# zaiisao/ConTEXTure-NeRF

Measured on AMD Instinct MI355X. Metric: UNet denoise steps/sec (CFG-batched SD2-depth UNet eval + PLMS update), higher is better.
Workload: dtype f16; 1 GPU; BASELINE configs[1]: 1 view @768^2 (latent 96^2), 50 PLMS steps (51 UNet evals), SD2-depth UNet fp16, CFG batch 2, guidance 10, random-init weights; mesh substitution napoleon.obj -> n/a for this stage (denoise loop only); latent=96, cfg_batch=2, ctx_len=77, views_per_rank=1, parallelism=view-shard x1

## Files before the change

contexture-nerf_amd/_lib.py:

```python
import ctypes as C
import os
import torch

_HERE = os.path.dirname(os.path.abspath(__file__))
LIB_PATH = os.path.join(_HERE, "libctxnerf.so")

_vp, _i32, _i64, _f32 = C.c_void_p, C.c_int32, C.c_int64, C.c_float

SIGNATURES = {
    "ctx_version": (_i32, []),
    "ctx_last_error": (C.c_char_p, []),
    "ctx_device_check": (_i32, []),
    "ctx_prepare_vertices": (_i32, [_vp, _vp, _vp, _vp, _i32, _i32, _i32, _vp, _vp, _vp, _vp, _vp]),
    "ctx_rasterize_ws_bytes": (_i64, [_i32, _i32, _i32, _i32]),
    "ctx_rasterize_fwd": (_i32, [_i32, _i32, _vp, _vp, _vp, _i32, _i32, _i32, _f32, _f32, _vp, _vp, _vp, _i64, _vp]),
    "ctx_rasterize_fused": (_i32, [_i32, _i32, _vp, _vp, _vp, _i32, _vp, _i32, _i32, _f32, _f32, _vp, _vp, _vp, _vp, _vp, _i64, _vp]),
    "ctx_normalize_depth_ws_bytes": (_i64, [_i32]),
    "ctx_normalize_depth": (_i32, [_vp, _i32, _i32, _vp, _vp, _vp, _vp]),
    "ctx_texture_mapping_fwd": (_i32, [_vp, _vp, _i32, _i32, _i32, _i32, _i32, _i32, _vp, _vp, _vp]),
    "ctx_texture_mapping_bwd": (_i32, [_vp, _vp, _i32, _i32, _i32, _i32, _vp, _vp, _vp]),
    "ctx_texmap_bwd_plan_bytes": (_i64, [_i32, _i32, _i32]),
    "ctx_texmap_bwd_plan": (_i32, [_vp, _vp, _i32, _i32, _i32, _vp, _vp]),
    "ctx_texture_mapping_bwd_binned_ws_bytes": (_i64, [_i32, _i32]),
    "ctx_texture_mapping_bwd_binned": (_i32, [_vp, _vp, _vp, _i32, _i32, _i32, _i32, _vp, _vp, _vp, _vp]),
    "ctx_texmap_plan_max_res": (_i32, []),
    "ctx_texmap_plan_stale": (_i32, [_vp, _vp]),
    "ctx_uv_scatter_fixed": (_i32, [_vp, _vp, _vp, _i32, _i32, _i32, _i32, _vp, _i32, _vp, _vp]),
    "ctx_fixed_to_float": (_i32, [_vp, _i64, _i32, _i32, _vp, _vp]),
    "ctx_uv_gather_ws_bytes": (_i64, [_i32, _i32]),
    "ctx_uv_gather_fixed": (_i32, [_vp, _vp, _vp, _vp, _vp, _vp, _vp, _i32, _i32, _i32, _i32, _i32, _i32, _i32, _vp, _vp, _i64, _vp]),
    "ctx_atlas_fill_ws_bytes": (_i64, [_i32]),
    "ctx_nearest_seed": (_i32, [_vp, _i32, _vp, _vp, _vp, _i64, _vp]),
    "ctx_atlas_fill": (_i32, [_vp, _vp, _vp, _i32, _i32, _i32, _vp, _vp, _vp, _i64, _vp]),
    "ctx_view_consistency_ws_bytes": (_i64, [_i32, _i32]),
    "ctx_view_consistency_fwd": (_i32, [_vp, _vp, _vp, _vp, _i32, _i32, _i32, _i32, _i32, _i32, _i32, _i32, _vp, _i64, _vp, _vp, _vp, _vp, _vp]),
    "ctx_view_consistency_bwd": (_i32, [_vp, _vp, _vp, _vp, _vp, _i32, _i32, _i32, _i32, _i32, _i32, _i32, _vp, _vp, _vp, _vp, _vp]),
    "ctx_texture_pack4": (_i32, [_vp, _i32, _i32, _vp, _vp]),
    "ctx_texture_mapping_packed_fwd": (_i32, [_vp, _vp, _i32, _i32, _i32, _i32, _i32, _vp, _vp, _vp]),
    "ctx_view_weights_max": (_i32, [_vp, _vp, _i32, _i32, _i32, _vp, _vp, _vp]),
    "ctx_view_weights_mask": (_i32, [_vp, _vp, _vp, _i32, _i32, _i32, _vp, _vp]),
    "ctx_face_view_map_ws_bytes": (_i64, [_i32, _i32, _i32]),
    "ctx_face_view_map": (_i32, [_vp, _i32, _i32, _i32, _vp, _vp, _vp, _vp]),
    "ctx_embed_fwd": (_i32, [_vp, _i64, _i32, _i32, _vp, _vp]),
    "ctx_uvmlp_packed_bytes": (_i64, [_i32, _i32, _i32, _i32, _i32]),
    "ctx_uvmlp_pack": (_i32, [_vp, _vp, _i32, _i32, _i32, _i32, _i32, _vp, _vp]),
    "ctx_uvmlp_fwd": (_i32, [_vp, _vp, _i64, _i32, _vp, _i32, _i32, _i32, _i32, _i32, _vp, _vp, _vp]),
    "ctx_uvmlp_saved_bytes": (_i64, [_i64, _i32, _i32, _i32]),
    "ctx_uvmlp_fwd_save": (_i32, [_vp, _vp, _i64, _i32, _vp, _i32, _i32, _i32, _i32, _i32, _i32, _vp, _vp, _vp, _vp]),
    "ctx_uvmlp_bwd_ws_bytes": (_i64, [_i64, _i32, _i32]),
    "ctx_uvmlp_bwd": (_i32, [_vp, _vp, _vp, _i64, _vp, _i32, _i32, _i32, _i32, _i32, _i32, _vp, _vp, _vp, _vp, _vp]),
    "ctx_uvmlp_fwd_emb": (_i32, [_vp, _i64, _vp, _i32, _i32, _i32, _i32, _i32, _vp, _vp, _vp]),
    "ctx_uvmlp_bwd_emb": (_i32, [_vp, _i64, _vp, _i32, _i32, _i32, _i32, _i32, _vp, _vp, _vp, _vp, _vp, _vp]),
    "ctx_texel_active_mark": (_i32, [_vp, _vp, _i32, _i32, _i32, _i32, _vp, _vp]),
    "ctx_texel_compact_ws_bytes": (_i64, [_i64]),
    "ctx_texel_compact": (_i32, [_vp, _i64, _vp, _vp, _vp, _vp]),
    "ctx_uvmlp_fwd_save_idx": (_i32, [_vp, _i64, _i32, _vp, _i32, _i32, _i32, _i32, _i32, _vp, _vp, _vp, _vp]),
    "ctx_uvmlp_bwd_idx": (_i32, [_vp, _vp, _vp, _i32, _vp, _i64, _vp, _i32, _i32, _i32, _i32, _i32, _vp, _vp, _vp, _vp, _vp]),
    "ctx_get_rays": (_i32, [_i32, _i32, _f32, _f32, _f32, _f32, _vp, _vp, _vp, _vp]),
    "ctx_raymarch_composite_fwd": (_i32, [_vp, _vp, _vp, _i64, _i32, _i32, _vp, _vp, _vp, _vp, _vp, _vp]),
    "ctx_raymarch_composite_fwd_noise": (_i32, [_vp, _vp, _vp, _vp, _i64, _i32, _i32, _vp, _vp, _vp, _vp, _vp, _vp]),
    "ctx_raymarch_composite_bwd": (_i32, [_vp, _vp, _vp, _vp, _i64, _i32, _i32, _vp, _vp, _vp, _vp, _vp, _vp, _vp]),
    "ctx_occ_mark": (_i32, [_vp, _vp, _vp, _i64, _i32, _vp, _i32, _f32, _f32, _f32, _f32, _f32, _f32, _vp, _vp]),
    "ctx_occ_points": (_i32, [_vp, _vp, _vp, _i64, _i32, _vp, _i64, _vp, _vp]),
    "ctx_occ_expand": (_i32, [_vp, _vp, _i64, _i64, _vp, _vp]),
    "ctx_occ_collect": (_i32, [_vp, _vp, _i64, _i64, _vp, _vp]),
    "ctx_occ_cell_points": (_i32, [_i32, _f32, _f32, _f32, _f32, _f32, _f32, _vp, _vp, _vp]),
    "ctx_occ_update": (_i32, [_vp, _vp, _vp, _i64, _f32, _f32, _vp]),
    "ctx_occ_voxelize": (_i32, [_vp, _vp, _i64, _i64, _i32, _f32, _f32, _f32, _f32, _f32, _f32, _vp, _vp]),
    "ctx_occ_dilate": (_i32, [_vp, _i32, _i32, _vp, _vp, _vp]),
    "ctx_occ_ray_spans": (_i32, [_vp, _vp, _i64, _f32, _f32, _vp, _i32, _f32, _f32, _f32, _f32, _f32, _f32, _f32, _f32, _f32, _f32, _f32, _f32,
                                 _vp, _vp, _vp]),
    "ctx_occ_march_count": (_i32, [_vp, _vp, _i64, _f32, _f32, _vp, _i32] + [_f32] * 13 + [_vp, _vp]),
    "ctx_occ_march_write": (_i32, [_vp, _vp, _i64, _f32, _f32, _vp, _i32] + [_f32] * 13 + [_vp, _vp, _i64, _vp, _vp, _vp, _vp, _vp]),
    "ctx_raymarch_packed_fwd": (_i32, [_vp, _vp, _vp, _vp, _vp, _vp, _i64, _i64, _i32, _vp, _vp, _vp, _vp, _vp, _vp]),
    "ctx_raymarch_packed_bwd": (_i32, [_vp, _vp, _vp, _vp, _vp, _vp, _i64, _i64, _i32, _vp, _vp, _vp, _vp, _vp, _vp, _vp]),
    "ctx_distortion_packed_fwd": (_i32, [_vp, _vp, _vp, _vp, _vp, _i64, _i64, _vp, _vp]),
    "ctx_distortion_packed_bwd": (_i32, [_vp, _vp, _vp, _vp, _vp, _i64, _i64, _vp, _vp, _vp]),
    "ctx_resample_packed": (_i32, [_vp, _vp, _vp, _vp, _vp, _vp, _i64, _i64, _i32, _vp, _vp, _i64, _vp, _vp, _vp, _vp, _vp]),
    "ctx_hashgrid_fwd": (_i32, [_vp, _i64, _vp, _i32, _i32, _i32, _vp, _vp, _vp, _vp, _vp]),
    "ctx_hashgrid_bwd_ws_bytes": (_i64, [_i32, _i32, _i32]),
    "ctx_hashgrid_bwd": (_i32, [_vp, _i64, _vp, _i32, _i32, _i32, _vp, _vp, _vp, _i32, _vp, _vp, _vp]),
    "ctx_hashgrid_bwd_pts_ws_bytes": (_i64, [_i64, _i32]),
    "ctx_hashgrid_bwd_pts": (_i32, [_vp, _i64, _vp, _vp, _i32, _i32, _i32, _vp, _vp, _vp, _vp, _vp, _vp]),
    "ctx_hashtex_fwd": (_i32, [_vp, _vp, _i64, _i32, _vp, _i32, _i32, _i32, _vp, _vp, _vp]),
    "ctx_hashtex_bwd_ws_bytes": (_i64, [_i32, _i32, _i32]),
    "ctx_hashtex_bwd": (_i32, [_vp, _vp, _i64, _i32, _vp, _i32, _i32, _i32, _vp, _i32, _vp, _vp, _vp]),
    "ctx_texture_head_fwd": (_i32, [_vp, _vp, _i64, _i64, _i32, _vp, _vp]),
    "ctx_texture_head_bwd": (_i32, [_vp, _vp, _vp, _vp, _i64, _i64, _i32, _vp, _vp]),
    "ctx_weighted_sum_packed": (_i32, [_vp, _vp, _vp, _i64, _i64, _i32, _vp, _vp]),
    "ctx_unet_create": (_vp, [_vp]),
    "ctx_unet_destroy": (None, [_vp]),
    "ctx_unet_param_count": (_i32, [_vp]),
    "ctx_unet_param_name": (C.c_char_p, [_vp, _i32]),
    "ctx_unet_param_shape": (_i32, [_vp, _i32, _vp]),
    "ctx_unet_weight_bytes": (_i64, [_vp]),
    "ctx_unet_workspace_bytes": (_i64, [_vp, _i32, _i32, _i32, _i32]),
    "ctx_unet_bind": (_i32, [_vp, _vp, _vp, _i64]),
    "ctx_unet_set_param": (_i32, [_vp, _i32, _vp, _vp]),
    "ctx_unet_forward": (_i32, [_vp, _vp, _vp, _vp, _i32, _i32, _i32, _i32, _vp, _vp]),
    "ctx_controlnet_create": (_vp, [_vp, _i32]),
    "ctx_controlnet_residual_bytes": (_i64, [_vp, _i32, _i32, _i32]),
    "ctx_controlnet_cond_cache_bytes": (_i64, [_vp, _i32, _i32, _i32]),
    "ctx_controlnet_forward": (_i32, [_vp, _vp, _vp, _vp, _vp, _vp, _i32, _i32, _i32, _i32, _i32, _vp, _vp]),
    "ctx_unet_set_residuals": (_i32, [_vp, _vp, C.c_float]),
    "ctx_unet_ref_bank_bytes": (_i64, [_vp, _i32, _i32, _i32]),
    "ctx_unet_workspace_bytes_ref": (_i64, [_vp, _i32, _i32, _i32, _i32, _i32, _i32]),
    "ctx_unet_forward_ref": (_i32, [_vp, _vp, _vp, _vp, _i32, _i32, _i32, _i32, _i32, _vp, _i32, _vp, _vp]),
    "ctx_unet_set_residual_fp32": (_i32, [_vp, _i32]),
    "ctx_unet_stats": (_i32, [_vp, _i32, _vp, _vp]),
    "ctx_unet_gn_epilogue_counts": (_i32, [_vp, _vp, _vp]),
    "ctx_unet_set_taps": (_i32, [_vp, _vp, _i64]),
    "ctx_unet_tap_count": (_i32, [_vp]),
    "ctx_unet_tap_info": (_i32, [_vp, _i32, _vp, _vp, _vp]),
    "ctx_vae_create": (_vp, [_vp]),
    "ctx_vae_destroy": (None, [_vp]),
    "ctx_vae_param_count": (_i32, [_vp]),
    "ctx_vae_param_name": (C.c_char_p, [_vp, _i32]),
    "ctx_vae_param_shape": (_i32, [_vp, _i32, _vp]),
    "ctx_vae_weight_bytes": (_i64, [_vp]),
    "ctx_vae_workspace_bytes": (_i64, [_vp, _i32, _i32, _i32]),
    "ctx_vae_bind": (_i32, [_vp, _vp, _vp, _i64]),
    "ctx_vae_set_param": (_i32, [_vp, _i32, _vp, _vp]),
    "ctx_vae_decode": (_i32, [_vp, _vp, _i32, _i32, _i32, _vp, _vp]),
    "ctx_vae_decoder_param_count": (_i32, [_vp]),
    "ctx_vae_encode_workspace_bytes": (_i64, [_vp, _i32, _i32, _i32]),
    "ctx_vae_encode": (_i32, [_vp, _vp, _i32, _i32, _i32, _vp, _vp]),
    "ctx_vae_flops": (C.c_double, [_vp]),
    "ctx_vae_encode_train_workspace_bytes": (_i64, [_vp, _i32, _i32, _i32]),
    "ctx_vae_encode_train": (_i32, [_vp, _vp, _i32, _i32, _i32, _vp, _vp]),
    "ctx_vae_encode_bwd": (_i32, [_vp, _vp, _f32, _vp, _vp]),
    "ctx_gemm_f16": (_i32, [_vp, _vp, _vp, _vp, _i32, _i32, _i32, _vp, _vp]),
    "ctx_conv3x3_f16": (_i32, [_vp, _vp, _vp, _vp, _vp, _i32, _i32, _i32, _i32, _i32, _i32, _i32, _vp, _vp]),
    "ctx_conv3x3_seg_f16": (_i32, [_vp, _vp, _vp, _vp, _vp, _vp, _i32, _i32, _i32, _i32, _i32, _vp, _vp, _i32, _i32, _vp, _vp, _i32, _i32,
                                   _vp, _i32, _vp, _vp]),
    "ctx_conv3x3_gn_f16": (_i32, [_vp, _vp, _vp, _vp, _vp, _vp, _i32, _i32, _i32, _i32, _i32, _vp, _i32, _i32, _i32, _vp, _vp, _vp, _vp]),
    "ctx_gemm_last_kernel": (None, [_vp, _vp]),
    "ctx_conv3x3_geom_f16": (_i32, [_vp, _vp, _vp, _vp, _i32, _i32, _i32, _i32, _i32, _i32, _i32, _i32, _i32, _vp, _i32, _vp, _vp]),
    "ctx_pack_conv3_dgrad_f16": (_i32, [_vp, _i32, _i32, _i32, _vp, _vp]),
    "ctx_pack_mat_dgrad_f16": (_i32, [_vp, _i32, _i32, _i32, _i32, _vp, _vp]),
    "ctx_groupnorm_bwd_ws_bytes": (_i64, [_i32, _i32]),
    "ctx_groupnorm_bwd_f16": (_i32, [_vp, _vp, _vp, _vp, _vp, _i32, _i32, _i32, _i32, _f32, _i32, _vp, _vp, _vp]),
    "ctx_softmax_rows_f16": (_i32, [_vp, _i32, _i32, _f32, _vp, _vp]),
    "ctx_softmax_bwd_rows_f16": (_i32, [_vp, _vp, _i32, _i32, _f32, _vp, _vp]),
    "ctx_quant_bwd_f16": (_i32, [_vp, _vp, _i32, _i32, _i64, _f32, _vp, _vp]),
    "ctx_conv_in_bwd_f16": (_i32, [_vp, _vp, _i32, _i32, _i32, _i32, _i32, _f32, _vp, _vp]),
    "ctx_conv_in_f16": (_i32, [_vp, _vp, _vp, _i32, _i32, _i32, _i32, _i32, _vp, _vp]),
    "ctx_conv_out_f16": (_i32, [_vp, _vp, _vp, _i32, _i32, _i32, _i32, _i32, _vp, _vp]),
    "ctx_gemv_f16": (_i32, [_vp, _vp, _vp, _i32, _i32, _i32, _i32, _i32, _vp, _vp]),
    "ctx_time_embed_f16": (_i32, [_vp, _i32, _i32, _vp, _vp]),
    "ctx_transpose_v_f16": (_i32, [_vp, _i32, _i32, _i32, _i32, _i32, _vp, _vp]),
    "ctx_concat_f16": (_i32, [_vp, _vp, _i64, _i32, _i32, _vp, _vp]),
    "ctx_concat_f32": (_i32, [_vp, _vp, _i64, _i32, _i32, _vp, _vp]),
    "ctx_f32_to_f16": (_i32, [_vp, _i64, _vp, _vp]),
    "ctx_f16_to_f32": (_i32, [_vp, _i64, _vp, _vp]),
    "ctx_conv_small_f16": (_i32, [_vp, _vp, _vp, _vp, _i32, _i32, _i32, _i32, _i32, _i32, _i32, _vp, _vp]),
    "ctx_add_scaled_f16": (_i32, [_vp, _vp, _f32, _i64, _vp]),
    "ctx_pointwise_f32": (_i32, [_vp, _vp, _vp, _i32, _i32, _i64, _i32, _vp, _vp]),
    "ctx_pack_fwd_f16": (_i32, [_vp, _i32, _i32, _i32, _vp, _vp]),
    "ctx_groupnorm_f16": (_i32, [_vp, _vp, _vp, _i32, _i32, _i32, _i32, _f32, _i32, _vp, _vp, _vp]),
    "ctx_groupnorm2_f16": (_i32, [_vp, _vp, _i32, _vp, _vp, _i32, _i32, _i32, _i32, _f32, _i32, _vp, _vp, _vp]),
    "ctx_groupnorm_apply_f16": (_i32, [_vp, _vp, _i32, _vp, _vp, _i32, _i32, _i32, _i32, _f32, _i32, _vp, _vp]),
    "ctx_groupnorm_slabs_f16": (_i32, [_vp, _i32, _vp, _vp, _vp, _i32, _vp, _vp, _i32, _i32, _i32, _i32, _f32, _i32, _vp, _vp]),
    "ctx_layernorm_f16": (_i32, [_vp, _vp, _vp, _i64, _i32, _f32, _vp, _vp]),
    "ctx_attention_ws_bytes": (_i64, [_i32, _i32, _i32]),
    "ctx_attention_f16": (_i32, [_vp, _vp, _vp, _i32, _i32, _i32, _i32, _i32, _i32, _f32, _vp, _i32, _vp, _vp]),
    "ctx_groupnorm_ws_bytes": (_i64, [_i32, _i32]),
    "ctx_geglu_f16": (_i32, [_vp, _i64, _i32, _vp, _vp]),
    "ctx_profile_begin": (_i32, []),
    "ctx_profile_end": (_i32, [_i32, _vp, _vp]),
    "ctx_bench_gemm": (C.c_float, [_vp, _vp, _vp, _vp, _i32, _i32, _i32, _vp, _i32, _i32, _i32, _i32, _i32, _i32, _vp, _i32, _i32, _vp]),
    "ctx_gemm_tune": (None, [_i32, _i32]),
    "ctx_attention_tune": (None, [_i32, _i32, _i32, _f32]),
    "ctx_probe_mfma": (_i32, [_i32, _vp, _vp, _vp, _vp]),
    "ctx_probe_stage": (C.c_float, [_i32, _i32, _i32, _i32, _i32, _vp, _vp, _vp]),
    "ctx_cfg_plms_step": (_i32, [_vp, _i64, _f32, _vp, _i32, _vp, _f32, _f32, _i32, _vp, _vp, _vp]),
}


class CtxError(RuntimeError):
    pass


_lib = None


def load():
    global _lib
    if _lib is None:
        if not os.path.exists(LIB_PATH):
            raise CtxError(f"{LIB_PATH} is missing: run `python -c 'import __graft_entry__ as g; g.build()'` "
                           "(hipcc --offload-arch=gfx950). There is no CPU fallback for this path.")
        lib = C.CDLL(LIB_PATH)
        for name, (res, args) in SIGNATURES.items():
            if not hasattr(lib, name) and os.environ.get("CTX_ALLOW_PARTIAL") == "1":
                continue
            fn = getattr(lib, name)
            fn.restype = res
            fn.argtypes = args
        _lib = lib
    return _lib


def check(rc):
    if rc != 0:
        raise CtxError(f"libctxnerf error {rc}: {load().ctx_last_error().decode()}")


def stream():
    return C.c_void_p(torch.cuda.current_stream().cuda_stream)


def ptr(t, dtype=None, name="tensor"):
    if t is None:
        return C.c_void_p(0)
    if not isinstance(t, torch.Tensor) or not t.is_cuda:
        raise CtxError(f"{name}: expected a device tensor (the HIP path has no CPU fallback), got "
                       f"{type(t).__name__} on {getattr(t, 'device', '?')}")
    if not t.is_contiguous():
        raise CtxError(f"{name}: tensor must be contiguous")
    if dtype is not None and t.dtype != dtype:
        raise CtxError(f"{name}: expected dtype {dtype}, got {t.dtype}")
    return C.c_void_p(t.data_ptr())


def f32c(t, device=None):
    t = t.to(dtype=torch.float32)
    if device is not None:
        t = t.to(device)
    return t.contiguous()
```

contexture-nerf_amd/csrc/attention.hip:

```cpp
#include "gemm_common.h"
#include <math.h>

#define AT_KB 64
#define AT_KROW 72
#define AT_VROW 68


struct AttnArgs {
    const f16 *Q, *K, *V;
    f16 *O;
    int Sq, Skv, heads;
    int q_stride, kv_stride, o_stride;
    float scale_log2e;
    float lazy;
};



typedef short at_s16x4 __attribute__((__vector_size__(4 * sizeof(short))));
__device__ __forceinline__ f16x4 at_tr16(const f16 *p)
{
    at_s16x4 v = __builtin_amdgcn_ds_read_tr16_b64_v4i16((__attribute__((address_space(3))) at_s16x4 *)p);
    return __builtin_bit_cast(f16x4, v);
}
struct AtNoIssue { __device__ __forceinline__ void operator()(int) const {} };
template <bool MASK, int NISSUE = 0, class Issue = AtNoIssue>
__device__ __forceinline__ void attn_tile(const f16 *__restrict__ Ks, const f16 *__restrict__ Vs, int k0, int Skv, int r, int h,
                                          int swz, int vlane, int vfq, float c, const f16x8 (&qf)[4], f32x16 (&o)[2], f32x16 &ls,
                                          float &m_run, float lazy, Issue iss = Issue())
{
    f32x16 s[2];
#pragma unroll
    for (int kb = 0; kb < 2; ++kb) {
#pragma unroll
        for (int q = 0; q < 16; ++q) s[kb][q] = 0.f;
        const f16 *kr = Ks + (kb * 32 + r) * 64;
#pragma unroll
        for (int ks = 0; ks < 4; ++ks) {
            f16x8 kf = *(const f16x8 *)(kr + ((2 * ks + h) ^ swz) * 8);
            s[kb] = __builtin_amdgcn_mfma_f32_32x32x16_f16(kf, qf[ks], s[kb], 0, 0, 0);
            if (kb * 4 + ks < NISSUE) iss(kb * 4 + ks);
        }
    }
    if (MASK) {
#pragma unroll
        for (int kb = 0; kb < 2; ++kb)
#pragma unroll
            for (int q = 0; q < 16; ++q) {
                int key = k0 + kb * 32 + (q & 3) + 8 * (q >> 2) + 4 * h;
                if (key >= Skv) s[kb][q] = -INFINITY;
            }
    }
    float mxa = fmaxf(s[0][0], s[0][1]), mxb = fmaxf(s[1][0], s[1][1]);
#pragma unroll
    for (int q = 2; q < 16; q += 2) {
        mxa = __builtin_fmaxf(__builtin_fmaxf(mxa, s[0][q]), s[0][q + 1]);
        mxb = __builtin_fmaxf(__builtin_fmaxf(mxb, s[1][q]), s[1][q + 1]);
    }
    float mx = fmaxf(mxa, mxb);
    mx = fmaxf(mx, __shfl_xor(mx, 32, 64)) * c;
    const float m_cand = fmaxf(m_run, mx);
    const bool move = __any(m_cand > m_run + lazy);
    const float m_new = move ? m_cand : m_run;
    typedef float at_f2 __attribute__((ext_vector_type(2)));
    const at_f2 c2 = {c, c}, nm2 = {-m_new, -m_new};
#pragma unroll
    for (int kb = 0; kb < 2; ++kb)
#pragma unroll
        for (int q = 0; q < 16; q += 2) {
            const at_f2 t = __builtin_elementwise_fma((at_f2){s[kb][q], s[kb][q + 1]}, c2, nm2);
            s[kb][q] = __builtin_amdgcn_exp2f(t[0]);
            s[kb][q + 1] = __builtin_amdgcn_exp2f(t[1]);
        }
    if (move) {
        const float alpha = __builtin_amdgcn_exp2f(m_run - m_new);
        asm volatile("s_nop 1\n\tv_mul_f32 %0, %0, %1" : "+v"(ls[0]) : "v"(alpha));
#pragma unroll
        for (int d = 0; d < 2; ++d)
#pragma unroll
            for (int q = 0; q < 16; ++q) asm volatile("v_mul_f32 %0, %0, %1" : "+v"(o[d][q]) : "v"(alpha));
    }
    m_run = m_new;
    const f16x8 ones = {1, 1, 1, 1, 1, 1, 1, 1};
#pragma unroll
    for (int kb = 0; kb < 2; ++kb)
#pragma unroll
        for (int st = 0; st < 2; ++st) {
            f16x8 pf;
#pragma unroll
            for (int j = 0; j < 8; ++j) pf[j] = (f16)s[kb][8 * st + j];
            const f16 *vk = Vs + (32 * kb + 16 * st + 4 * h) * 64 + vlane;
#pragma unroll
            for (int d = 0; d < 2; ++d) {
                const int co = ((4 * d) ^ vfq) * 8;
                f16x4 v0 = at_tr16(vk + co), v1 = at_tr16(vk + 8 * 64 + co);
                f16x8 vf = __builtin_shufflevector(v0, v1, 0, 1, 2, 3, 4, 5, 6, 7);
                o[d] = __builtin_amdgcn_mfma_f32_32x32x16_f16(vf, pf, o[d], 0, 0, 0);
            }
            ls = __builtin_amdgcn_mfma_f32_32x32x16_f16(ones, pf, ls, 0, 0, 0);
        }
}

template <int AT_NS, int NW, bool SPREAD = true>
__global__ __launch_bounds__(64 * NW, NW == 8 ? 4 : 1) void k_attention_dma(AttnArgs a)
{
    __shared__ __attribute__((aligned(16))) f16 ring[AT_NS * 2 * 64 * 64];
    const int tid = threadIdx.x, lane = tid & 63, wave = __builtin_amdgcn_readfirstlane(tid >> 6);
    const int r = lane & 31, h = lane >> 5;
    const int b = blockIdx.z, hd = blockIdx.y;
    const int q0 = blockIdx.x * (32 * NW) + wave * 32;
    const int qrow = q0 + r;
    const bool qok = qrow < a.Sq;
    constexpr int PI = 8 / NW;
    constexpr int G = 2 * PI;

    f16x8 qf[4];
    const f16x8 zero8 = {0, 0, 0, 0, 0, 0, 0, 0};
    {
        const f16 *qp = a.Q + ((size_t)b * a.Sq + (qok ? qrow : 0)) * a.q_stride + hd * 64 + 8 * h;
#pragma unroll
        for (int ks = 0; ks < 4; ++ks) qf[ks] = qok ? *(const f16x8 *)(qp + ks * 16) : zero8;
    }
    f32x16 o[2];
#pragma unroll
    for (int d = 0; d < 2; ++d)
#pragma unroll
        for (int q = 0; q < 16; ++q) o[d][q] = 0.f;
    f32x16 ls;
#pragma unroll
    for (int q = 0; q < 16; ++q) ls[q] = 0.f;
    float m_run = -INFINITY;

    const int ntiles = (a.Skv + AT_KB - 1) / AT_KB;
    const int lr = lane >> 3, pc = lane & 7;
    const f16 *kp[PI], *vp[PI];
    int krow[PI];
#pragma unroll
    for (int i = 0; i < PI; ++i) {
        int row = 8 * (wave + NW * i) + lr;
        int lc = (pc ^ ((row >> 1) & 7)) * 8;
        krow[i] = row;
        kp[i] = a.K + ((size_t)b * a.Skv + row) * a.kv_stride + hd * 64 + lc;
        vp[i] = a.V + ((size_t)b * a.Skv + row) * a.kv_stride + hd * 64 + ((pc ^ (((row >> 1) & 1) << 2)) * 8);
    }
    int issued = 0;
    auto issue = [&](int buf) {
        f16 *Ks = ring + buf * (2 * 64 * 64);
        f16 *Vs = Ks + 64 * 64;
        const int k0 = issued * AT_KB;
#pragma unroll
        for (int i = 0; i < PI; ++i) {
            const f16 *src = (k0 + krow[i] < a.Skv) ? kp[i] : ctx_zero_page;
            __builtin_amdgcn_global_load_lds((gptr_t)src, (lptr_t)(Ks + (wave + NW * i) * 512), 16, 0, 0);
            kp[i] += (size_t)AT_KB * a.kv_stride;
        }
#pragma unroll
        for (int i = 0; i < PI; ++i) {
            const f16 *src = (k0 + krow[i] < a.Skv) ? vp[i] : ctx_zero_page;
            __builtin_amdgcn_global_load_lds((gptr_t)src, (lptr_t)(Vs + (wave + NW * i) * 512), 16, 0, 0);
            vp[i] += (size_t)AT_KB * a.kv_stride;
        }
        ++issued;
    };
    auto issue_piece = [&](int buf, int idx) {
        f16 *Ks = ring + buf * (2 * 64 * 64);
        f16 *Vs = Ks + 64 * 64;
        const int k0 = issued * AT_KB;
        const int i = idx < PI ? idx : idx - PI;
        const f16 *&gp = idx < PI ? kp[i] : vp[i];
        const f16 *src = (k0 + krow[i] < a.Skv) ? gp : ctx_zero_page;
        __builtin_amdgcn_global_load_lds((gptr_t)src, (lptr_t)((idx < PI ? Ks : Vs) + (wave + NW * i) * 512), 16, 0, 0);
        gp += (size_t)AT_KB * a.kv_stride;
    };
#pragma unroll
    for (int p = 0; p < AT_NS - 1; ++p)
        if (p < ntiles) issue(p);

    const int swz = (r >> 1) & 7;
    const int vq = (lane & 15) >> 2, vfq = ((vq >> 1) & 1) << 2;
    const int vlane = vq * 64 + (((2 * ((lane >> 4) & 1) + ((lane & 3) >> 1)) ^ 0) * 8) + (lane & 1) * 4;
    const float c = a.scale_log2e;
    const int nfull = a.Skv / AT_KB;
    int slot = 0;
    int t = 0;
    for (; t < nfull && t + AT_NS - 1 < ntiles; ++t) {
        asm volatile("s_waitcnt vmcnt(%0)" ::"n"((AT_NS - 2) * G) : "memory");
        __builtin_amdgcn_sched_barrier(0);
        ctx_barrier();
        const int ibuf = slot == 0 ? AT_NS - 1 : slot - 1;
        const f16 *Ks = ring + slot * (2 * 64 * 64);
        if (SPREAD) {
            attn_tile<false, G>(Ks, Ks + 64 * 64, t * AT_KB, a.Skv, r, h, swz, vlane, vfq, c, qf, o, ls, m_run, a.lazy, [&](int idx) { issue_piece(ibuf, idx); });
            ++issued;
        } else {
            issue(ibuf);
            attn_tile<false>(Ks, Ks + 64 * 64, t * AT_KB, a.Skv, r, h, swz, vlane, vfq, c, qf, o, ls, m_run, a.lazy);
        }
        slot = slot + 1 == AT_NS ? 0 : slot + 1;
    }
    for (; t < nfull; ++t) {
        const int newer = issued - 1 - t;
        if (AT_NS >= 4 && newer >= 2) asm volatile("s_waitcnt vmcnt(%0)" ::"n"(2 * G) : "memory");
        else if (newer >= 1) asm volatile("s_waitcnt vmcnt(%0)" ::"n"(G) : "memory");
        else asm volatile("s_waitcnt vmcnt(0)" ::: "memory");
        __builtin_amdgcn_sched_barrier(0);
        ctx_barrier();
        if (issued < ntiles) issue(slot == 0 ? AT_NS - 1 : slot - 1);
        const f16 *Ks = ring + slot * (2 * 64 * 64);
        attn_tile<false>(Ks, Ks + 64 * 64, t * AT_KB, a.Skv, r, h, swz, vlane, vfq, c, qf, o, ls, m_run, a.lazy);
        slot = slot + 1 == AT_NS ? 0 : slot + 1;
    }
    if (nfull < ntiles) {
        asm volatile("s_waitcnt vmcnt(0)" ::: "memory");
        ctx_barrier();
        const f16 *Ks = ring + slot * (2 * 64 * 64);
        attn_tile<true>(Ks, Ks + 64 * 64, nfull * AT_KB, a.Skv, r, h, swz, vlane, vfq, c, qf, o, ls, m_run, a.lazy);
    }
    if (qok) {
        float inv = 1.0f / ls[0];
        f16 *op = a.O + ((size_t)b * a.Sq + qrow) * a.o_stride + hd * 64;
#pragma unroll
        for (int d = 0; d < 2; ++d)
#pragma unroll
            for (int g = 0; g < 4; ++g) {
                f16x4 v;
#pragma unroll
                for (int j = 0; j < 4; ++j) v[j] = (f16)(o[d][4 * g + j] * inv);
                *(f16x4 *)(op + d * 32 + 8 * g + 4 * h) = v;
            }
    }
}

template <int NS, int NW, bool SPREAD = true>
static void attn_launch(const AttnArgs &a, int B, bool report, hipStream_t s)
{
    constexpr auto kern = k_attention_dma<NS, NW, SPREAD>;
    if (report) {
        int nb = 0;
        hipFuncAttributes fa;
        (void)hipOccupancyMaxActiveBlocksPerMultiprocessor(&nb, kern, 64 * NW, 0);
        (void)hipFuncGetAttributes(&fa, (const void *)kern);
        fprintf(stderr, "[ctx] attention: %d blocks/CU by the occupancy API, %d VGPRs, %zu B static LDS\n", nb, fa.numRegs, fa.sharedSizeBytes);
    }
    ctx_launch<kern>(1, dim3(cdiv(a.Sq, 32 * NW), a.heads, B), dim3(64 * NW), 0, s, a);
}

struct AttnTune { int ns, nw8, spread; float lazy; };
static AttnTune g_attn_force = {-1, -1, -1, -1.f};
static const AttnTune &attn_tune_env()
{
    static const AttnTune env = [] {
        AttnTune t;
        t.ns = ctx_env_int("CTX_ATTN_NS", 3);
        t.nw8 = ctx_env_int("CTX_ATTN_NW8", -1);
        t.spread = ctx_env_int("CTX_ATTN_SPREAD", 1);
        const char *e = getenv("CTX_ATTN_LAZY");
        t.lazy = e ? (float)atof(e) : 8.0f;
        if (!(t.lazy >= 0.f && t.lazy <= 12.f)) t.lazy = 8.0f;
        return t;
    }();
    return env;
}

extern "C" void ctx_attention_tune(int32_t ns, int32_t nw8, int32_t spread, float lazy)
{
    g_attn_force.ns = ns; g_attn_force.nw8 = nw8; g_attn_force.spread = spread; g_attn_force.lazy = lazy;
}

int ctx_attention_core(const f16 *Q, const f16 *K, const f16 *V, int B, int Sq, int Skv, int heads, int q_stride,
                       int kv_stride, float scale, f16 *O, int o_stride, hipStream_t s)
{
    AttnArgs a;
    a.Q = Q; a.K = K; a.V = V; a.O = O; a.Sq = Sq; a.Skv = Skv; a.heads = heads;
    a.q_stride = q_stride; a.kv_stride = kv_stride; a.o_stride = o_stride;
    a.scale_log2e = scale * 1.4426950408889634f;
    const AttnTune &tu = attn_tune_env();
    const float lazy = g_attn_force.lazy >= 0.f ? g_attn_force.lazy : tu.lazy;
    a.lazy = lazy >= 0.f && lazy <= 12.f ? lazy : 8.0f;
    const int ns = g_attn_force.ns >= 0 ? g_attn_force.ns : tu.ns;
    const int nw8 = g_attn_force.nw8 >= 0 ? g_attn_force.nw8 : tu.nw8;
    const bool w8 = nw8 == 1 || (nw8 < 0 && Sq >= 1024 && Sq < 4096 && Skv >= 1024);
    const int spread = g_attn_force.spread >= 0 ? g_attn_force.spread : tu.spread;
    static int dbg = -1;
    bool report = false;
    if (dbg < 0) { dbg = ctx_env_int("CTX_ATTN_DEBUG", 0); report = dbg != 0; }
    if (w8) {
        if (ns == 2) attn_launch<2, 8>(a, B, report, s); else if (ns == 4) attn_launch<4, 8>(a, B, report, s);
        else if (spread) attn_launch<3, 8>(a, B, report, s); else attn_launch<3, 8, false>(a, B, report, s);
    } else {
        if (ns == 2) attn_launch<2, 4>(a, B, report, s); else if (ns == 4) attn_launch<4, 4>(a, B, report, s);
        else if (spread) attn_launch<3, 4>(a, B, report, s); else attn_launch<3, 4, false>(a, B, report, s);
    }
    hipError_t e = hipGetLastError();
    if (e != hipSuccess) {
        ctx_set_error("attention launch failed: %s", hipGetErrorString(e));
        return CTX_E_LAUNCH;
    }
    return CTX_OK;
}

extern "C" int64_t ctx_attention_ws_bytes(int32_t B, int32_t Skv, int32_t heads)
{
    (void)B; (void)Skv; (void)heads;
    return 256;
}

extern "C" int32_t ctx_attention_f16(const void *Q, const void *K, const void *V, int32_t B, int32_t Sq, int32_t Skv,
                                     int32_t heads, int32_t q_stride, int32_t kv_stride, float scale, void *O,
                                     int32_t o_stride, void *vt_ws, ctx_stream_t stream)
{
    (void)vt_ws;
    CTX_REQUIRE(Q && K && V && O, "attention: null pointer");
    CTX_REQUIRE(B > 0 && Sq > 0 && Skv > 0 && heads > 0 && q_stride % 8 == 0 && kv_stride % 8 == 0 && o_stride % 4 == 0 &&
                    q_stride >= heads * 64 && kv_stride >= heads * 64 && o_stride >= heads * 64,
                "attention: bad strides/sizes (head_dim is fixed at 64)");
    return ctx_attention_core((const f16 *)Q, (const f16 *)K, (const f16 *)V, B, Sq, Skv, heads, q_stride, kv_stride, scale, (f16 *)O,
                              o_stride, (hipStream_t)stream);
}
```

include/ctx_nerf.h:

```cpp
#ifndef CTX_NERF_H
#define CTX_NERF_H
#include <stdint.h>
#ifdef __cplusplus
extern "C" {
#endif

#define CTX_OK 0
#define CTX_E_ARG (-1)
#define CTX_E_LAUNCH (-2)
#define CTX_E_STATE (-3)

typedef void *ctx_stream_t;

int32_t ctx_version(void);
const char *ctx_last_error(void);
int32_t ctx_device_check(void);

int32_t ctx_prepare_vertices(const float *verts, const int64_t *faces, const float *cam,
                             const float *proj3, int32_t B, int32_t V, int32_t F,
                             float *fv_cam, float *fv_img, float *fnorm,
                             void *ws , ctx_stream_t stream);

int64_t ctx_rasterize_ws_bytes(int32_t H, int32_t W, int32_t B, int32_t F);
int32_t ctx_rasterize_fwd(int32_t H, int32_t W, const float *face_z, const float *face_xy,
// ... 172 lines not shown

int32_t ctx_weighted_sum_packed(const float *weights, const float *values, const int64_t *ray_off, int64_t R, int64_t n, int32_t C,
                                float *out, ctx_stream_t stream);

typedef struct ctx_unet ctx_unet_t;
typedef struct {
    int32_t in_channels, out_channels;
    int32_t n_levels;
    int32_t block_out_channels[4];
    int32_t heads[4];
    int32_t down_attn[4], up_attn[4];
    int32_t layers_per_block;
    int32_t cross_attention_dim;
    int32_t groups;
    float norm_eps;
} ctx_unet_config_t;

ctx_unet_t *ctx_unet_create(const ctx_unet_config_t *cfg);
void ctx_unet_destroy(ctx_unet_t *u);
int32_t ctx_unet_param_count(const ctx_unet_t *u);
const char *ctx_unet_param_name(const ctx_unet_t *u, int32_t i);
int32_t ctx_unet_param_shape(const ctx_unet_t *u, int32_t i, int64_t shape4[4]);
int64_t ctx_unet_weight_bytes(const ctx_unet_t *u);
int64_t ctx_unet_workspace_bytes(const ctx_unet_t *u, int32_t B, int32_t H, int32_t W, int32_t ctx_len);
int32_t ctx_unet_bind(ctx_unet_t *u, void *weights, void *workspace, int64_t workspace_bytes);
int32_t ctx_unet_set_param(ctx_unet_t *u, int32_t i, const float *src, ctx_stream_t stream);
int32_t ctx_unet_forward(ctx_unet_t *u, const float *sample, const float *timestep, const float *ctx,
                         int32_t B, int32_t H, int32_t W, int32_t ctx_len, float *out, ctx_stream_t stream);
int64_t ctx_unet_ref_bank_bytes(const ctx_unet_t *u, int32_t B, int32_t H, int32_t W);
int64_t ctx_unet_workspace_bytes_ref(const ctx_unet_t *u, int32_t B, int32_t H, int32_t W, int32_t ctx_len, int32_t mode,
                                     int32_t ref_row0);
int32_t ctx_unet_forward_ref(ctx_unet_t *u, const float *sample, const float *timestep, const float *ctx,
                             int32_t B, int32_t H, int32_t W, int32_t ctx_len, int32_t mode, void *bank, int32_t ref_row0,
                             float *out, ctx_stream_t stream);
ctx_unet_t *ctx_controlnet_create(const ctx_unet_config_t *cfg, int32_t cond_channels);
int64_t ctx_controlnet_residual_bytes(const ctx_unet_t *cn, int32_t B, int32_t H, int32_t W);
int64_t ctx_controlnet_cond_cache_bytes(const ctx_unet_t *cn, int32_t B, int32_t H, int32_t W);
int32_t ctx_controlnet_forward(ctx_unet_t *cn, const float *sample, const float *timestep, const float *ctx,
                               const float *cond , void *cond_cache, int32_t cache_valid,
                               int32_t B, int32_t H, int32_t W, int32_t ctx_len, void *residuals, ctx_stream_t stream);
int32_t ctx_unet_set_residuals(ctx_unet_t *u, const void *residuals , float scale);
int32_t ctx_unet_set_residual_fp32(ctx_unet_t *u, int32_t on);
int32_t ctx_unet_stats(const ctx_unet_t *u, int32_t klass, int64_t *launches, double *flops);
int32_t ctx_unet_gn_epilogue_counts(const ctx_unet_t *u, int64_t *from_producer, int64_t *from_slabs);
int32_t ctx_unet_set_taps(ctx_unet_t *u, void *buf, int64_t capacity);
int32_t ctx_unet_tap_count(const ctx_unet_t *u);
int32_t ctx_unet_tap_info(const ctx_unet_t *u, int32_t i, int64_t *offset, int32_t *rows, int32_t *channels);

typedef struct ctx_vae ctx_vae_t;
typedef struct {
    int32_t latent_channels, out_channels;
    int32_t n_levels;
    int32_t block_out_channels[4];
    int32_t layers_per_block;
    int32_t groups;
} ctx_vae_config_t;
ctx_vae_t *ctx_vae_create(const ctx_vae_config_t *cfg);
void ctx_vae_destroy(ctx_vae_t *v);
int32_t ctx_vae_param_count(const ctx_vae_t *v);
const char *ctx_vae_param_name(const ctx_vae_t *v, int32_t i);
int32_t ctx_vae_param_shape(const ctx_vae_t *v, int32_t i, int64_t shape4[4]);
int64_t ctx_vae_weight_bytes(const ctx_vae_t *v);
int64_t ctx_vae_workspace_bytes(const ctx_vae_t *v, int32_t B, int32_t H, int32_t W);
int32_t ctx_vae_bind(ctx_vae_t *v, void *weights, void *workspace, int64_t workspace_bytes);
int32_t ctx_vae_set_param(ctx_vae_t *v, int32_t i, const float *src, ctx_stream_t stream);
int32_t ctx_vae_decode(ctx_vae_t *v, const float *latents, int32_t B, int32_t H, int32_t W, float *image, ctx_stream_t stream);
int32_t ctx_vae_decoder_param_count(const ctx_vae_t *v);
int64_t ctx_vae_encode_workspace_bytes(const ctx_vae_t *v, int32_t B, int32_t H, int32_t W);
int32_t ctx_vae_encode(ctx_vae_t *v, const float *image, int32_t B, int32_t H, int32_t W, float *moments, ctx_stream_t stream);
double ctx_vae_flops(const ctx_vae_t *v);
int64_t ctx_vae_encode_train_workspace_bytes(const ctx_vae_t *v, int32_t B, int32_t H, int32_t W);
int32_t ctx_vae_encode_train(ctx_vae_t *v, const float *image, int32_t B, int32_t H, int32_t W, float *moments, ctx_stream_t stream);
int32_t ctx_vae_encode_bwd(ctx_vae_t *v, const float *grad_moments, float gscale, float *grad_image, ctx_stream_t stream);

int32_t ctx_gemm_f16(const void *A, const void *Wt, const void *bias, const void *residual,
                     int32_t M, int32_t N, int32_t K, void *C, ctx_stream_t stream);
int32_t ctx_conv3x3_f16(const void *x, const void *w, const void *bias, const void *rowbias,
                        const void *residual, int32_t B, int32_t H, int32_t W, int32_t Cin,
                        int32_t Cout, int32_t stride, int32_t upsample, void *y, ctx_stream_t stream);
int32_t ctx_conv3x3_seg_f16(const void *x, const void *w, const void *bias, const void *bias2, const void *rowbias,
                            const void *residual, int32_t B, int32_t H, int32_t W, int32_t Cin, int32_t Cout,
                            const void *xa, const void *wa, int32_t Ca, int32_t ldwa, const void *xb, const void *wb,
                            int32_t Cb, int32_t ldwb, void *part, int32_t splitk, void *y, ctx_stream_t stream);
int32_t ctx_conv3x3_gn_f16(const void *x, const void *w, const void *bias, const void *bias2, const void *rowbias,
                           const void *residual, int32_t B, int32_t H, int32_t W, int32_t Cin, int32_t Cout, void *part,
                           int32_t splitk, int32_t keep_slabs, int32_t groups, void *gn_part, int32_t *slots, void *y,
                           ctx_stream_t stream);
void ctx_gemm_last_kernel(int32_t *tile, int32_t *use8);
int32_t ctx_conv3x3_geom_f16(const void *x, const void *w, const void *bias, const void *residual, int32_t B, int32_t H, int32_t W,
                             int32_t Cin, int32_t Cout, int32_t stride, int32_t upsample, int32_t poff, int32_t zins, void *part,
                             int32_t splitk, void *y, ctx_stream_t stream);
int32_t ctx_pack_conv3_dgrad_f16(const float *src, int32_t Cout, int32_t Cin, int32_t pad, void *dst, ctx_stream_t stream);
int32_t ctx_pack_mat_dgrad_f16(const float *src, int32_t out, int32_t in, int32_t ld, int32_t col, void *dst, ctx_stream_t stream);
int64_t ctx_groupnorm_bwd_ws_bytes(int32_t B, int32_t groups);
int32_t ctx_groupnorm_bwd_f16(const void *x, const void *dy, const void *gamma, const void *beta, const void *add, int32_t B, int32_t HW,
                              int32_t C, int32_t groups, float eps, int32_t silu, void *dx, void *ws, ctx_stream_t stream);
int32_t ctx_softmax_rows_f16(const void *s, int32_t rows, int32_t n, float scale, void *p, ctx_stream_t stream);
int32_t ctx_softmax_bwd_rows_f16(const void *P, const void *dP, int32_t rows, int32_t n, float scale, void *dS, ctx_stream_t stream);
int32_t ctx_quant_bwd_f16(const float *g, const void *w, int32_t B, int32_t C, int64_t HW, float gscale, void *d, ctx_stream_t stream);
int32_t ctx_conv_in_bwd_f16(const void *dy, const void *w_pack, int32_t B, int32_t H, int32_t W, int32_t C, int32_t Cimg, float inv_gscale,
                            float *dimg, ctx_stream_t stream);
int32_t ctx_conv_in_f16(const float *x, const void *w_pack, const void *bias, int32_t B, int32_t Cin, int32_t H, int32_t W, int32_t Cout,
                        void *y, ctx_stream_t stream);
int32_t ctx_conv_out_f16(const void *x, const void *w, const void *bias, int32_t B, int32_t H, int32_t W, int32_t C, int32_t Cout,
                         float *out, ctx_stream_t stream);
int32_t ctx_gemv_f16(const void *x, const void *w, const void *bias, int32_t Bm, int32_t N, int32_t K, int32_t silu_in, int32_t silu_out,
                     void *out, ctx_stream_t stream);
int32_t ctx_time_embed_f16(const float *t, int32_t B, int32_t dim, void *out, ctx_stream_t stream);
int32_t ctx_transpose_v_f16(const void *v, int32_t B, int32_t S, int32_t ld, int32_t heads, int32_t Sp, void *vt, ctx_stream_t stream);
int32_t ctx_concat_f16(const void *a, const void *b, int64_t M, int32_t Ca, int32_t Cb, void *y, ctx_stream_t stream);
int32_t ctx_concat_f32(const float *a, const float *b, int64_t M, int32_t Ca, int32_t Cb, float *y, ctx_stream_t stream);
int32_t ctx_f32_to_f16(const float *x, int64_t n, void *y, ctx_stream_t stream);
int32_t ctx_f16_to_f32(const void *x, int64_t n, float *y, ctx_stream_t stream);
int32_t ctx_conv_small_f16(const float *x32, const void *x16, const void *w, const void *bias, int32_t B, int32_t H, int32_t W, int32_t Cin,
                           int32_t Cout, int32_t stride, int32_t silu, void *y, ctx_stream_t stream);
int32_t ctx_add_scaled_f16(void *dst, const void *src, float scale, int64_t n, ctx_stream_t stream);
int32_t ctx_pointwise_f32(const void *x, const void *w, const void *b, int32_t B, int32_t C, int64_t HW, int32_t nhwc16, float *y,
                          ctx_stream_t stream);
int32_t ctx_pack_fwd_f16(const float *src, int32_t kind, int32_t a, int32_t b, void *dst, ctx_stream_t stream);
int64_t ctx_groupnorm_ws_bytes(int32_t B, int32_t groups);
int32_t ctx_groupnorm_f16(const void *x, const void *gamma, const void *beta, int32_t B, int32_t HW,
                          int32_t C, int32_t groups, float eps, int32_t silu, void *y, void *stats_ws,
                          ctx_stream_t stream);
int32_t ctx_groupnorm2_f16(const void *xa, const void *xb, int32_t Ca, const void *gamma, const void *beta, int32_t B,
                           int32_t HW, int32_t C, int32_t groups, float eps, int32_t silu, void *y, void *stats_ws,
                           ctx_stream_t stream);
int32_t ctx_groupnorm_apply_f16(const void *x, const void *part, int32_t slots, const void *gamma, const void *beta, int32_t B,
                                int32_t HW, int32_t C, int32_t groups, float eps, int32_t silu, void *y, ctx_stream_t stream);
int32_t ctx_groupnorm_slabs_f16(const void *part, int32_t splitk, const void *bias, const void *bias2, const void *rowbias,
                                int32_t ldrb, const void *gamma, const void *beta, int32_t B, int32_t HW, int32_t C,
                                int32_t groups, float eps, int32_t silu, void *y, ctx_stream_t stream);
int32_t ctx_layernorm_f16(const void *x, const void *gamma, const void *beta, int64_t rows, int32_t C,
                          float eps, void *y, ctx_stream_t stream);
int64_t ctx_attention_ws_bytes(int32_t B, int32_t Skv, int32_t heads);
int32_t ctx_attention_f16(const void *Q, const void *K, const void *V, int32_t B, int32_t Sq, int32_t Skv,
                          int32_t heads, int32_t q_stride, int32_t kv_stride, float scale, void *O,
                          int32_t o_stride, void *vt_ws, ctx_stream_t stream);
int32_t ctx_geglu_f16(const void *h, int64_t M, int32_t C4, void *y, ctx_stream_t stream);

int32_t ctx_cfg_plms_step(const float *eps_pair, int64_t n, float guidance, float *ets, int32_t head,
                          const float *coef4, float sample_coeff, float eps_coeff, int32_t mode,
                          float *cur_sample_ws, float *x, ctx_stream_t stream);

int32_t ctx_profile_begin(void);
int32_t ctx_profile_end(int32_t klass, double *total_ms , int64_t *count );

float ctx_bench_gemm(const void *A, const void *Wt, const void *bias, const void *residual, int32_t M, int32_t N, int32_t K,
                     void *C, int32_t conv_B, int32_t conv_H, int32_t conv_W, int32_t conv_Cin, int32_t conv_flags, int32_t epi,
                     void *part, int32_t splitk, int32_t iters, ctx_stream_t stream);

void ctx_gemm_tune(int32_t tile, int32_t gemm8);

void ctx_attention_tune(int32_t ns, int32_t nw8, int32_t spread, float lazy);

int32_t ctx_probe_mfma(int32_t which, const void *A, const void *Bt, float *C, ctx_stream_t stream);

float ctx_probe_stage(int32_t mode, int32_t waves, int32_t u, int32_t iters, int32_t shared_region, const void *src, void *sink,
                      ctx_stream_t stream);

#ifdef __cplusplus
}
#endif
#endif
```

Measured before the change: 122.5 steps/s.

## Add warp-specialized loader wave variant for DMA-ring attention kernel

Adds an attention kernel variant in which a fifth wave streams K/V tiles into the LDS ring with global_load_lds. The four compute waves then only wait on barriers and run the MFMA tile math, with no interleaved load issue or vmcnt waits. A heuristic turns it on for mid-sized grids (Skv>=512, 192-384 workgroups), which covers the 48x48 and 24x24 self-attention layers; an env var and a tune entry point can override it. The goal is to decouple memory issue from compute. The cost is an extra wave per workgroup, different occupancy bounds, and replacing the 8-wave path that was used for those shapes.

```diff
diff --git a/contexture-nerf_amd/_lib.py b/contexture-nerf_amd/_lib.py
--- a/contexture-nerf_amd/_lib.py
+++ b/contexture-nerf_amd/_lib.py
@@ -171,6 +171,7 @@
     "ctx_bench_gemm": (C.c_float, [_vp, _vp, _vp, _vp, _i32, _i32, _i32, _vp, _i32, _i32, _i32, _i32, _i32, _i32, _vp, _i32, _i32, _vp]),
     "ctx_gemm_tune": (None, [_i32, _i32]),
     "ctx_attention_tune": (None, [_i32, _i32, _i32, _f32]),
+    "ctx_attention_tune_loader": (None, [_i32]),
     "ctx_probe_mfma": (_i32, [_i32, _vp, _vp, _vp, _vp]),
     "ctx_probe_stage": (C.c_float, [_i32, _i32, _i32, _i32, _i32, _vp, _vp, _vp]),
     "ctx_cfg_plms_step": (_i32, [_vp, _i64, _f32, _vp, _i32, _vp, _f32, _f32, _i32, _vp, _vp, _vp]),
diff --git a/contexture-nerf_amd/csrc/attention.hip b/contexture-nerf_amd/csrc/attention.hip
--- a/contexture-nerf_amd/csrc/attention.hip
+++ b/contexture-nerf_amd/csrc/attention.hip
@@ -101,13 +101,70 @@
         }
 }
 
-template <int AT_NS, int NW, bool SPREAD = true>
-__global__ __launch_bounds__(64 * NW, NW == 8 ? 4 : 1) void k_attention_dma(AttnArgs a)
-{
+template <int AT_NS>
+__device__ __forceinline__ void attn_loader(const AttnArgs &a, f16 *ring, int lane, int b, int hd, int ntiles)
+{
+    const int lr = lane >> 3, pc = lane & 7;
+    const unsigned rowoff = (unsigned)(lr * a.kv_stride) * 2u;
+    const unsigned koff[2] = {rowoff + (unsigned)((pc ^ (lr >> 1)) * 16), rowoff + (unsigned)((pc ^ (lr >> 1) ^ 4) * 16)};
+    const unsigned voff = rowoff + (unsigned)((pc ^ (((lr >> 1) & 1) << 2)) * 16);
+    const size_t piece = (size_t)8 * a.kv_stride * 2, tile = (size_t)AT_KB * a.kv_stride * 2;
+    const char *kt = (const char *)(a.K + (size_t)b * a.Skv * a.kv_stride + hd * 64);
+    const char *vt = (const char *)(a.V + (size_t)b * a.Skv * a.kv_stride + hd * 64);
+    int issued = 0;
+    auto issue = [&](int buf) {
+        f16 *Ks = ring + buf * (2 * 64 * 64);
+        f16 *Vs = Ks + 64 * 64;
+        const int k0 = issued * AT_KB;
+        if (k0 + AT_KB <= a.Skv) {
+#pragma unroll
+            for (int i = 0; i < 8; ++i) __builtin_amdgcn_global_load_lds((gptr_t)(kt + i * piece + koff[i & 1]), (lptr_t)(Ks + i * 512), 16, 0, 0);
+#pragma unroll
+            for (int i = 0; i < 8; ++i) __builtin_amdgcn_global_load_lds((gptr_t)(vt + i * piece + voff), (lptr_t)(Vs + i * 512), 16, 0, 0);
+        } else {
+#pragma unroll
+            for (int i = 0; i < 8; ++i) {
+                const char *src = (k0 + 8 * i + lr < a.Skv) ? kt + i * piece + koff[i & 1] : (const char *)ctx_zero_page;
+                __builtin_amdgcn_global_load_lds((gptr_t)src, (lptr_t)(Ks + i * 512), 16, 0, 0);
+            }
+#pragma unroll
+            for (int i = 0; i < 8; ++i) {
+                const char *src = (k0 + 8 * i + lr < a.Skv) ? vt + i * piece + voff : (const char *)ctx_zero_page;
+                __builtin_amdgcn_global_load_lds((gptr_t)src, (lptr_t)(Vs + i * 512), 16, 0, 0);
+            }
+        }
+        kt += tile; vt += tile;
+        ++issued;
+    };
+#pragma unroll
+    for (int p = 0; p < AT_NS - 1; ++p)
+        if (p < ntiles) issue(p);
+    int slot = 0;
+    for (int t = 0; t < ntiles; ++t) {
+        const int newer = issued - 1 - t;
+        if (AT_NS >= 4 && newer >= 2) asm volatile("s_waitcnt vmcnt(32)" ::: "memory");
+        else if (AT_NS >= 3 && newer >= 1) asm volatile("s_waitcnt vmcnt(16)" ::: "memory");
+        else asm volatile("s_waitcnt vmcnt(0)" ::: "memory");
+        ctx_barrier();
+        if (issued < ntiles) issue(slot == 0 ? AT_NS - 1 : slot - 1);
+        slot = slot + 1 == AT_NS ? 0 : slot + 1;
+    }
+}
+
+template <int AT_NS, int NW, bool SPREAD = true, bool LOADER = false>
+__global__ __launch_bounds__(64 * (NW + LOADER), NW == 8 ? 4 : LOADER ? (AT_NS == 4 ? 3 : 4) : 1) void k_attention_dma(AttnArgs a)
+{
+    static_assert(!LOADER || NW == 4, "the loader form is the 4-wave workgroup plus one wave");
     __shared__ __attribute__((aligned(16))) f16 ring[AT_NS * 2 * 64 * 64];
     const int tid = threadIdx.x, lane = tid & 63, wave = __builtin_amdgcn_readfirstlane(tid >> 6);
     const int r = lane & 31, h = lane >> 5;
     const int b = blockIdx.z, hd = blockIdx.y;
+    if constexpr (LOADER) {
+        if (wave == NW) {
+            attn_loader<AT_NS>(a, ring, lane, b, hd, (a.Skv + AT_KB - 1) / AT_KB);
+            return;
+        }
+    }
     const int q0 = blockIdx.x * (32 * NW) + wave * 32;
     const int qrow = q0 + r;
     const bool qok = qrow < a.Sq;
@@ -172,9 +229,11 @@
         __builtin_amdgcn_global_load_lds((gptr_t)src, (lptr_t)((idx < PI ? Ks : Vs) + (wave + NW * i) * 512), 16, 0, 0);
         gp += (size_t)AT_KB * a.kv_stride;
     };
-#pragma unroll
-    for (int p = 0; p < AT_NS - 1; ++p)
-        if (p < ntiles) issue(p);
+    if constexpr (!LOADER) {
+#pragma unroll
+        for (int p = 0; p < AT_NS - 1; ++p)
+            if (p < ntiles) issue(p);
+    }
 
     const int swz = (r >> 1) & 7;
     const int vq = (lane & 15) >> 2, vfq = ((vq >> 1) & 1) << 2;
@@ -183,38 +242,54 @@
     const int nfull = a.Skv / AT_KB;
     int slot = 0;
     int t = 0;
-    for (; t < nfull && t + AT_NS - 1 < ntiles; ++t) {
-        asm volatile("s_waitcnt vmcnt(%0)" ::"n"((AT_NS - 2) * G) : "memory");
-        __builtin_amdgcn_sched_barrier(0);
-        ctx_barrier();
-        const int ibuf = slot == 0 ? AT_NS - 1 : slot - 1;
-        const f16 *Ks = ring + slot * (2 * 64 * 64);
-        if (SPREAD) {
-            attn_tile<false, G>(Ks, Ks + 64 * 64, t * AT_KB, a.Skv, r, h, swz, vlane, vfq, c, qf, o, ls, m_run, a.lazy, [&](int idx) { issue_piece(ibuf, idx); });
-            ++issued;
-        } else {
-            issue(ibuf);
+    if constexpr (LOADER) {
+        for (; t < nfull; ++t) {
+            __builtin_amdgcn_sched_barrier(0);
+            ctx_barrier();
+            const f16 *Ks = ring + slot * (2 * 64 * 64);
             attn_tile<false>(Ks, Ks + 64 * 64, t * AT_KB, a.Skv, r, h, swz, vlane, vfq, c, qf, o, ls, m_run, a.lazy);
-        }
-        slot = slot + 1 == AT_NS ? 0 : slot + 1;
-    }
-    for (; t < nfull; ++t) {
-        const int newer = issued - 1 - t;
-        if (AT_NS >= 4 && newer >= 2) asm volatile("s_waitcnt vmcnt(%0)" ::"n"(2 * G) : "memory");
-        else if (newer >= 1) asm volatile("s_waitcnt vmcnt(%0)" ::"n"(G) : "memory");
-        else asm volatile("s_waitcnt vmcnt(0)" ::: "memory");
-        __builtin_amdgcn_sched_barrier(0);
-        ctx_barrier();
-        if (issued < ntiles) issue(slot == 0 ? AT_NS - 1 : slot - 1);
-        const f16 *Ks = ring + slot * (2 * 64 * 64);
-        attn_tile<false>(Ks, Ks + 64 * 64, t * AT_KB, a.Skv, r, h, swz, vlane, vfq, c, qf, o, ls, m_run, a.lazy);
-        slot = slot + 1 == AT_NS ? 0 : slot + 1;
-    }
-    if (nfull < ntiles) {
-        asm volatile("s_waitcnt vmcnt(0)" ::: "memory");
-        ctx_barrier();
-        const f16 *Ks = ring + slot * (2 * 64 * 64);
-        attn_tile<true>(Ks, Ks + 64 * 64, nfull * AT_KB, a.Skv, r, h, swz, vlane, vfq, c, qf, o, ls, m_run, a.lazy);
+            slot = slot + 1 == AT_NS ? 0 : slot + 1;
+        }
+        if (nfull < ntiles) {
+            __builtin_amdgcn_sched_barrier(0);
+            ctx_barrier();
+            const f16 *Ks = ring + slot * (2 * 64 * 64);
+            attn_tile<true>(Ks, Ks + 64 * 64, nfull * AT_KB, a.Skv, r, h, swz, vlane, vfq, c, qf, o, ls, m_run, a.lazy);
+        }
+    } else {
+        for (; t < nfull && t + AT_NS - 1 < ntiles; ++t) {
+            asm volatile("s_waitcnt vmcnt(%0)" ::"n"((AT_NS - 2) * G) : "memory");
+            __builtin_amdgcn_sched_barrier(0);
+            ctx_barrier();
+            const int ibuf = slot == 0 ? AT_NS - 1 : slot - 1;
+            const f16 *Ks = ring + slot * (2 * 64 * 64);
+            if (SPREAD) {
+                attn_tile<false, G>(Ks, Ks + 64 * 64, t * AT_KB, a.Skv, r, h, swz, vlane, vfq, c, qf, o, ls, m_run, a.lazy, [&](int idx) { issue_piece(ibuf, idx); });
+                ++issued;
+            } else {
+                issue(ibuf);
+                attn_tile<false>(Ks, Ks + 64 * 64, t * AT_KB, a.Skv, r, h, swz, vlane, vfq, c, qf, o, ls, m_run, a.lazy);
+            }
+            slot = slot + 1 == AT_NS ? 0 : slot + 1;
+        }
+        for (; t < nfull; ++t) {
+            const int newer = issued - 1 - t;
+            if (AT_NS >= 4 && newer >= 2) asm volatile("s_waitcnt vmcnt(%0)" ::"n"(2 * G) : "memory");
+            else if (newer >= 1) asm volatile("s_waitcnt vmcnt(%0)" ::"n"(G) : "memory");
+            else asm volatile("s_waitcnt vmcnt(0)" ::: "memory");
+            __builtin_amdgcn_sched_barrier(0);
+            ctx_barrier();
+            if (issued < ntiles) issue(slot == 0 ? AT_NS - 1 : slot - 1);
+            const f16 *Ks = ring + slot * (2 * 64 * 64);
+            attn_tile<false>(Ks, Ks + 64 * 64, t * AT_KB, a.Skv, r, h, swz, vlane, vfq, c, qf, o, ls, m_run, a.lazy);
+            slot = slot + 1 == AT_NS ? 0 : slot + 1;
+        }
+        if (nfull < ntiles) {
+            asm volatile("s_waitcnt vmcnt(0)" ::: "memory");
+            ctx_barrier();
+            const f16 *Ks = ring + slot * (2 * 64 * 64);
+            attn_tile<true>(Ks, Ks + 64 * 64, nfull * AT_KB, a.Skv, r, h, swz, vlane, vfq, c, qf, o, ls, m_run, a.lazy);
+        }
     }
     if (qok) {
         float inv = 1.0f / ls[0];
@@ -231,22 +306,23 @@
     }
 }
 
-template <int NS, int NW, bool SPREAD = true>
+template <int NS, int NW, bool SPREAD = true, bool LOADER = false>
 static void attn_launch(const AttnArgs &a, int B, bool report, hipStream_t s)
 {
-    constexpr auto kern = k_attention_dma<NS, NW, SPREAD>;
+    constexpr auto kern = k_attention_dma<NS, NW, SPREAD, LOADER>;
+    constexpr int threads = 64 * (NW + LOADER);
     if (report) {
         int nb = 0;
         hipFuncAttributes fa;
-        (void)hipOccupancyMaxActiveBlocksPerMultiprocessor(&nb, kern, 64 * NW, 0);
+        (void)hipOccupancyMaxActiveBlocksPerMultiprocessor(&nb, kern, threads, 0);
         (void)hipFuncGetAttributes(&fa, (const void *)kern);
         fprintf(stderr, "[ctx] attention: %d blocks/CU by the occupancy API, %d VGPRs, %zu B static LDS\n", nb, fa.numRegs, fa.sharedSizeBytes);
     }
-    ctx_launch<kern>(1, dim3(cdiv(a.Sq, 32 * NW), a.heads, B), dim3(64 * NW), 0, s, a);
-}
-
-struct AttnTune { int ns, nw8, spread; float lazy; };
-static AttnTune g_attn_force = {-1, -1, -1, -1.f};
+    ctx_launch<kern>(1, dim3(cdiv(a.Sq, 32 * NW), a.heads, B), dim3(threads), 0, s, a);
+}
+
+struct AttnTune { int ns, nw8, spread; float lazy; int loader; };
+static AttnTune g_attn_force = {-1, -1, -1, -1.f, -1};
 static const AttnTune &attn_tune_env()
 {
     static const AttnTune env = [] {
@@ -257,6 +333,7 @@
         const char *e = getenv("CTX_ATTN_LAZY");
         t.lazy = e ? (float)atof(e) : 8.0f;
         if (!(t.lazy >= 0.f && t.lazy <= 12.f)) t.lazy = 8.0f;
+        t.loader = ctx_env_int("CTX_ATTN_LOADER", -1);
         return t;
     }();
     return env;
@@ -266,6 +343,8 @@
 {
     g_attn_force.ns = ns; g_attn_force.nw8 = nw8; g_attn_force.spread = spread; g_attn_force.lazy = lazy;
 }
+
+extern "C" void ctx_attention_tune_loader(int32_t loader) { g_attn_force.loader = loader; }
 
 int ctx_attention_core(const f16 *Q, const f16 *K, const f16 *V, int B, int Sq, int Skv, int heads, int q_stride,
                        int kv_stride, float scale, f16 *O, int o_stride, hipStream_t s)
@@ -284,7 +363,13 @@
     static int dbg = -1;
     bool report = false;
     if (dbg < 0) { dbg = ctx_env_int("CTX_ATTN_DEBUG", 0); report = dbg != 0; }
-    if (w8) {
+    const int ldsw = g_attn_force.loader >= 0 ? g_attn_force.loader : tu.loader;
+    const long nwg = (long)cdiv(Sq, 128) * heads * B;
+    const bool loader = nw8 != 1 && kv_stride < (1 << 24) && (ldsw == 1 || (ldsw < 0 && Skv >= 512 && nwg >= 192 && nwg <= 384));
+    if (loader) {
+        if (ns == 2) attn_launch<2, 4, true, true>(a, B, report, s); else if (ns == 4) attn_launch<4, 4, true, true>(a, B, report, s);
+        else attn_launch<3, 4, true, true>(a, B, report, s);
+    } else if (w8) {
         if (ns == 2) attn_launch<2, 8>(a, B, report, s); else if (ns == 4) attn_launch<4, 8>(a, B, report, s);
         else if (spread) attn_launch<3, 8>(a, B, report, s); else attn_launch<3, 8, false>(a, B, report, s);
     } else {
diff --git a/include/ctx_nerf.h b/include/ctx_nerf.h
--- a/include/ctx_nerf.h
+++ b/include/ctx_nerf.h
@@ -348,6 +348,7 @@
 void ctx_gemm_tune(int32_t tile, int32_t gemm8);
 
 void ctx_attention_tune(int32_t ns, int32_t nw8, int32_t spread, float lazy);
+void ctx_attention_tune_loader(int32_t loader);
 
 int32_t ctx_probe_mfma(int32_t which, const void *A, const void *Bt, float *C, ctx_stream_t stream);
 
```

After: 122.9 steps/s (median of 6 runs). About the same (+0.4%).
